# salute-developers/GigaAM

Measured on AMD Instinct MI355X. Metric: RTFx v2_ctc batch32x20s (log-mel + encoder + greedy decode), higher is better.
Workload: dtype f32 (GEMMs: 3-term split on fp16 MFMA, fp32 accumulate)

## Files before the change

### gigaam_amd/_lib.py

```python
from __future__ import annotations

import ctypes as C
import os
from typing import Optional

_HERE = os.path.dirname(os.path.abspath(__file__))
LIB_NAME = "libgigaam_hip.so"
LIB_PATH = os.path.join(_HERE, LIB_NAME)

SUBS_CONV2D, SUBS_CONV1D = 0, 1
ATT_ROTARY, ATT_REL_POS = 0, 1
NORM_BATCH, NORM_LAYER = 0, 1
HEAD_NONE, HEAD_CTC, HEAD_RNNT, HEAD_EMO = 0, 1, 2, 3
DTYPE_F32, DTYPE_F16, DTYPE_BF16, DTYPE_F64, DTYPE_I64 = 0, 1, 2, 3, 4
GEMM_F32, GEMM_F16X3, GEMM_F16 = 0, 1, 2
PF_CLASSES = ["gemm", "conv2", "attn", "norm", "convmod", "stem", "frontend", "decode", "misc", "align_bt", "align_out"]


class GamConfig(C.Structure):
    _fields_ = [(n, C.c_int32) for n in (
        "sample_rate", "n_mels", "hop_length", "win_length", "n_fft", "center",
        "feat_in", "n_layers", "d_model", "subsampling", "subs_kernel_size", "subsampling_factor",
        "ff_expansion_factor", "self_attention_model", "n_heads", "pos_emb_max_len",
        "conv_norm_type", "conv_kernel_size",
# ... 36 lines not shown
    "gam_rnnt_beam_nbest": (C.c_int, [_P, _P, _P, C.c_int, C.c_int64, C.c_int, C.c_int, C.c_int, _P, _P, _P, _P, _P, _P, _P]),
    "gam_op_rnnt_beam_nbest": (C.c_int, [_P, _P, _P, C.c_int, C.c_int64, C.c_int, C.c_int, C.c_int, _P, _P, _P, _P, _P, _P, _P]),
    "gam_rnnt_beam": (C.c_int, [_P, _P, _P, C.c_int, C.c_int64, C.c_int, C.c_int, _P, _P, _P, _P, _P, _P]),
    "gam_op_rnnt_beam": (C.c_int, [_P, _P, _P, C.c_int, C.c_int64, C.c_int, C.c_int, _P, _P, _P, _P, _P, _P]),
    "gam_rnnt_align": (C.c_int, [_P, _P, _P, C.c_int, C.c_int64, _P, _P, C.c_int, _P, _P, _P, _P, _P]),
    "gam_op_rnnt_align": (C.c_int, [_P, _P, _P, C.c_int, C.c_int64, _P, _P, C.c_int, _P, _P, _P, _P, _P, _P]),
    "gam_op_rnnt_lattice_align": (C.c_int, [_P, _P, _P, C.c_int, C.c_int64, C.c_int, _P, _P, C.c_int, _P, _P, _P, _P, _P]),
    "gam_set_rnnt_align_workspace": (C.c_int, [_P, C.c_int64]),
    "gam_ctc_confidence": (C.c_int, [_P, _P, _P, C.c_int, C.c_int64, _P, _P, _P, C.c_int, C.c_int, C.c_int, _P, _P, _P, _P]),
    "gam_op_ctc_confidence": (C.c_int, [_P, _P, _P, C.c_int, C.c_int64, C.c_int, _P, _P, _P, C.c_int, C.c_int, C.c_int, _P, _P, _P, _P]),
    "gam_rnnt_confidence": (C.c_int, [_P, _P, _P, C.c_int, C.c_int64, _P, _P, _P, C.c_int, C.c_int, _P, _P, _P]),
    "gam_op_rnnt_confidence": (C.c_int, [_P, _P, _P, C.c_int, C.c_int64, _P, _P, _P, C.c_int, C.c_int, _P, _P, _P]),
    "gam_emo_probs": (C.c_int, [_P, _P, _P, C.c_int, C.c_int64, _P, _P]),
    "gam_rnnt_predict": (C.c_int, [_P, _P, _P, _P, C.c_int, _P, _P, _P, _P]),
    "gam_rnnt_joint": (C.c_int, [_P, _P, _P, C.c_int, C.c_int, C.c_int, _P, _P]),
    "gam_set_gemm_mode": (C.c_int, [_P, C.c_int]),
    "gam_get_gemm_mode": (C.c_int, [_P]),
    "gam_set_rnnt_cluster": (C.c_int, [_P, C.c_int]),
    "gam_get_rnnt_cluster": (C.c_int, [_P]),
    "gam_debug_buffer_hash": (C.c_int, [_P, C.c_int, C.POINTER(C.c_uint64), C.POINTER(C.c_int64)]),
    "gam_range_flag": (C.c_int, [_P, C.POINTER(C.c_int), _P]),
    "gam_range_flag_fetch": (C.c_int, [_P, _P, _P]),
    "gam_op_gemm": (C.c_int, [_P, _P, _P, _P, _P, C.c_int, C.c_int, C.c_int, C.c_int, _P]),
    "gam_op_attention": (C.c_int, [_P, _P, _P, _P, _P, _P, C.c_int, C.c_int, C.c_int, _P]),
    "gam_op_attention_ex": (C.c_int, [_P, _P, _P, _P, C.c_int64, _P, _P, _P, C.c_int, C.c_int, C.c_int, C.c_int, _P, _P, _P, _P]),
    "gam_tune_sp": (C.c_int, [C.c_int, C.c_int, C.c_int]),
    "gam_plan_sp": (C.c_int, [C.c_int, C.c_int, C.c_int, C.c_int, C.POINTER(C.c_int), C.POINTER(C.c_int), C.POINTER(C.c_int)]),
    "gam_plan_sp_ex": (C.c_int, [C.c_int, C.c_int, C.c_int, C.c_int, C.POINTER(C.c_int), C.POINTER(C.c_int), C.POINTER(C.c_int), C.POINTER(C.c_int)]),
    "gam_tune_sp_stages": (C.c_int, [C.c_int]),
    "gam_profile_enable": (C.c_int, [_P, C.c_int]),
    "gam_profile_pause": (C.c_int, [_P, C.c_int]),
    "gam_profile_read": (C.c_int, [_P, C.c_int, C.POINTER(C.c_double), C.POINTER(C.c_int64), C.POINTER(C.c_double)]),
    "gam_profile_read_bytes": (C.c_int, [_P, C.c_int, C.POINTER(C.c_double)]),
    "gam_last_error": (C.c_char_p, [_P]),
    "gam_comm_unique_id": (C.c_int, [C.c_char_p]),
    "gam_comm_create": (C.c_int, [C.c_char_p, C.c_int, C.c_int, C.c_int, C.POINTER(_P)]),
    "gam_comm_world": (C.c_int, [_P]),
    "gam_gather_ids": (C.c_int, [_P, _P, _P, _P, _P, C.c_int, C.c_int, _P, _P, _P, _P, _P]),
    "gam_comm_last_error": (C.c_char_p, [_P]),
    "gam_comm_destroy": (None, [_P]),
}

_lib: Optional[C.CDLL] = None


class GigaAMHipError(RuntimeError):
# ... 23 lines not shown
```

### gigaam_amd/csrc/gam_api.hip

```cpp
#include <hip/hip_runtime.h>

#include <algorithm>
#include <cmath>
#include <cstdarg>
#include <cstdio>
#include <cstring>
#include <map>
#include <string>
#include <vector>

#include "../../include/gigaam_hip.h"
#include "gam_align.h"
#include "gam_align_long.h"
#include "gam_kws.h"
#include "gam_attn.h"
#include "gam_beam.h"
#include "gam_rnnt_beam.h"
#include "gam_attn16.h"
#include "gam_comm.h"
#include "gam_common.h"
#include "gam_convmod.h"
#include "gam_decode.h"
#include "gam_rnnt_align.h"
#include "gam_confidence.h"
// ... 2294 lines not shown
  ProfScope ps(h, s, GAM_PF_DECODE, (double)rows * V * 8.0);
  hipLaunchKernelGGL(gam_log_softmax_kernel, dim3(gam_cdiv((long)rows, 4)), dim3(256), 0, s, h->jl.p, log_probs, (int)rows, V);
  HIPCHK(h, hipGetLastError());
  return 0;
}

int gam_emo_probs(gam_handle* h, const float* encoded, const int32_t* enc_len, int B, int64_t Tp, float* probs,
                  void* stream) {
  if (!h) return -1;
  if (h->cfg.head_type != GAM_HEAD_EMO || !h->has_head) return fail(h, -1, "model has no emotion head");
  if (B <= 0 || Tp <= 0 || !encoded || !probs) return fail(h, -1, "bad emotion-head arguments");
  HIPCHK(h, hipSetDevice(h->device));
  hipStream_t s = (hipStream_t)stream;
  const int D = h->cfg.d_model, NC = h->cfg.num_classes;
  ProfScope ps(h, s, GAM_PF_DECODE, (double)B * D * Tp * 4.0);
  hipLaunchKernelGGL(gam_emo_head_kernel, dim3(B), dim3(256), (size_t)(D + NC) * sizeof(float), s, encoded, enc_len,
                     h->emo_w, h->emo_b, probs, D, (int)Tp, NC);
  HIPCHK(h, hipGetLastError());
  return 0;
}

int gam_op_gemm(gam_handle* h, const float* A, const float* W, const float* bias, float* C, int M, int N, int K, int act,
                void* stream) {
  if (!h) return -1;
  HIPCHK(h, hipSetDevice(h->device));
  GamGemmArgs g = gemm_args(A, K, W, bias, C, N, M, N, K);
  hipStream_t s = (hipStream_t)stream;
  if (!split_mode(h) || K % 32 != 0 || N % 4 != 0) return gemm(h, s, g, act);
  const size_t wn = (size_t)N * K, an = (size_t)M * K;
  W16 w16;
  if (int r = ensure(h, h->op_sp, wn + 64)) return r;
  hipLaunchKernelGGL(gam_to_sp32_kernel, dim3((int)std::min<size_t>((wn / 4 + 255) / 256, 4096)), dim3(256), 0, s, W,
                     (_Float16*)h->op_sp.p, wn / 4, (const float*)nullptr, K);
  w16.sp = (_Float16*)h->op_sp.p;
  if (int r = ensure(h, h->op_rs, (size_t)M + 64)) return r;
  hipLaunchKernelGGL(gam_rowscale_kernel, dim3(gam_cdiv(M, 4)), dim3(256), 0, s, A, h->op_rs.p, M, K, (long)K);
  g.a_rs = h->op_rs.p;
  if (int r = ensure(h, h->aplanes, an + 64)) return r;
  g.Asp = (const _Float16*)h->aplanes.p;
  g.a_fmt = (h->gemm_mode == GAM_GEMM_F16 && K % 64 == 0) ? 2 : 1;
  if (g.a_fmt == 2) {
    if (int r = ensure(h, h->op_planes, wn / 2 + 64)) return r;
    w16.h16 = (_Float16*)h->op_planes.p;
    hipLaunchKernelGGL(gam_to_h16_kernel, dim3((int)std::min<size_t>((wn / 4 + 255) / 256, 4096)), dim3(256), 0, s, W, w16.h16,
                       wn / 4, (const float*)nullptr, K);
    hipLaunchKernelGGL(gam_to_h16_kernel, dim3((int)std::min<size_t>((an / 4 + 255) / 256, 8192)), dim3(256), 0, s, A,
                       (_Float16*)h->aplanes.p, an / 4, (const float*)h->op_rs.p, K);
  } else {
    hipLaunchKernelGGL(gam_to_sp32_kernel, dim3((int)std::min<size_t>((an / 4 + 255) / 256, 8192)), dim3(256), 0, s, A,
// ... 169 lines not shown
```

### gigaam_amd/csrc/gam_gemm_sp.h

```cpp
#pragma once
#include "gam_gemm.h"
#include <type_traits>
#if defined(GAM_SP_INSTRUMENT) && GAM_SP_INSTRUMENT
#include <algorithm>
#include <vector>
#endif

#ifndef GAM_SP_INSTRUMENT
#define GAM_SP_INSTRUMENT 0
#endif
#define GAM_SP_DBG(g) (GAM_SP_INSTRUMENT ? (g).dbg : 0)
#if GAM_SP_INSTRUMENT
#define GAM_SP_TL(i)                                                                  \
  if ((GAM_SP_DBG(g) & 16) && g.tlog != nullptr && threadIdx.x == 0) {                        \
    g.tlog[(size_t)lid * 8 + (i)] = wall_clock64();                                   \
    if ((i) == 1 || (i) == 2) g.tlog[(size_t)lid * 8 + 4 + (i)] = clock64();          \
    if ((i) == 0) g.tlog[(size_t)lid * 8 + 7] = blockIdx.x;                            \
  }
#else
#define GAM_SP_TL(i)
#endif

template <int MT, int NW, int NS = 2>
struct GamGemmSpCfg {
  static constexpr int BM = 64 * MT;
  static constexpr int BN = 64 * NW;
  static constexpr int NWAVES = 2 * NW;
  static constexpr int NT = 64 * NWAVES;
  static constexpr int A_BYTES = BM * 128;
  static constexpr int W_BYTES = BN * 128;
  static constexpr int STAGE = A_BYTES + W_BYTES;
  static constexpr int SMEM = NS * STAGE;
  static constexpr int NAI = BM / 8 / NWAVES;
  static constexpr int NWI = BN / 8 / NWAVES;
};

template <int ACT, int MT, int NW, int NS = 2, bool H16 = false>
__global__ __launch_bounds__(128 * NW, NW == 2 ? 2 : 1) void gam_gemm_sp_kernel(GamGemmArgs g) {
  extern __shared__ __attribute__((aligned(16))) unsigned char gam_smem_sp[];
  using Cfg = GamGemmSpCfg<MT, NW, NS>;
  constexpr int BM = Cfg::BM, BN = Cfg::BN, NAI = Cfg::NAI, NWI = Cfg::NWI, NWAVES = Cfg::NWAVES;
  typedef __attribute__((address_space(3))) void* lds_ptr_t;
  typedef const __attribute__((address_space(1))) void* glb_ptr_t;

  const int tid = threadIdx.x;
  const int lane = tid & 63;
  const int wave = __builtin_amdgcn_readfirstlane(tid >> 6);
  const int wm = wave / NW, wn = wave % NW;

  const int nbn = (g.N + BN - 1) / BN;
  const int total = gridDim.x;
  const int q8 = total >> 3, r8 = total & 7;
  const int bid = blockIdx.x;
  const int xcd = bid & 7;
  const int lid = (xcd < r8 ? xcd * (q8 + 1) : r8 * (q8 + 1) + (xcd - r8) * q8) + (bid >> 3);
  int tm = lid / nbn, tn = lid % nbn;
  if (g.skip_pad) {
    tm = bid / nbn;
    tn = bid % nbn;
// ... 6 lines not shown
  }
  const int m0 = tm * BM;
  const int n0 = tn * BN;
  if (g.skip_pad && g.lens != nullptr) {
    const int mlast = m0 + BM - 1 < g.M ? m0 + BM - 1 : g.M - 1;
    const int b0 = m0 / g.rpb;
    if (b0 == mlast / g.rpb && (m0 - b0 * g.rpb) / g.fdiv >= g.lens[b0]) return;
  }
  GAM_SP_TL(0);

  auto a_row_off = [&](int m) -> size_t {
    m = m < g.M ? m : g.M - 1;
    if (g.a_mode == 0) return (size_t)m * (size_t)g.lda;
    const int fr = m / g.conv_f2, ff = m - fr * g.conv_f2;
    return ((size_t)fr * 2 * g.conv_fp + 2 * ff) * (size_t)g.conv_c;
  };
  const size_t a_tile0 = a_row_off(m0);
  const unsigned char* Ab = reinterpret_cast<const unsigned char*>(g.n_switch > 0 && n0 >= g.n_switch ? g.Asp2 : g.Asp) + a_tile0 * 4;
  const unsigned char* Wb = reinterpret_cast<const unsigned char*>(g.Wsp) + (size_t)n0 * (size_t)g.K * 4;
  unsigned a_src[NAI], w_src[NWI];
#pragma unroll
  for (int i = 0; i < NAI; ++i) {
    const int row = 8 * (wave + NWAVES * i) + (lane >> 3);
    const int slot = (lane & 7) ^ ((row >> 1) & 7);
    a_src[i] = (unsigned)((a_row_off(m0 + row) - a_tile0) * 4) + slot * 16;
  }
#pragma unroll
  for (int i = 0; i < NWI; ++i) {
    const int row = 8 * (wave + NWAVES * i) + (lane >> 3);
    const int slot = (lane & 7) ^ ((row >> 1) & 7);
    int n = n0 + row;
    n = n < g.N ? n : g.N - 1;
    w_src[i] = (unsigned)(n - n0) * (unsigned)g.K * 4u + slot * 16;
  }

  f32x16 acc[MT][2];
#pragma unroll
  for (int i = 0; i < MT; ++i)
#pragma unroll
    for (int j = 0; j < 2; ++j)
#pragma unroll
      for (int r = 0; r < 16; ++r) acc[i][j][r] = 0.f;

  const int nslice = g.splitk > 1 ? g.splitk : 1;
  const int nk = g.K / 32 / nslice;
  const int kt_first = (nslice > 1 ? (int)blockIdx.y : 0) * nk, kt_end = kt_first + nk;
  int d_kt = kt_first, d_c0 = 0, d_kw = 0, d_kh = 0;
  if (g.a_mode != 0) {
    const int cb = kt_first / 9, t9 = kt_first - cb * 9;
    d_c0 = 32 * cb; d_kh = t9 / 3; d_kw = t9 - d_kh * 3;
  }
  auto dma_ka = [&]() -> size_t {
    if (g.a_mode == 0) return (size_t)d_kt * 128;
    return (((size_t)d_kh * g.conv_fp + d_kw) * (size_t)g.conv_c + d_c0) * 4;
  };
  auto dma_advance = [&]() {
    if (d_kt + 1 >= kt_end) return;
    ++d_kt;
    if (g.a_mode == 0) return;
    if (++d_kw == 3) {
      d_kw = 0;
      if (++d_kh == 3) { d_kh = 0; d_c0 += 32; }
    }
  };
  auto issue = [&](int stage) {
    unsigned char* sb = gam_smem_sp + stage * Cfg::STAGE + wave * 1024;
    const unsigned char* ab = Ab + dma_ka();
    const unsigned char* wb = Wb + (size_t)d_kt * 128;
#pragma unroll
    for (int i = 0; i < NAI; ++i)
      __builtin_amdgcn_global_load_lds((glb_ptr_t)(ab + a_src[i]), (lds_ptr_t)(sb + i * (NWAVES * 1024)), 16, 0, 0);
#pragma unroll
    for (int i = 0; i < NWI; ++i)
      __builtin_amdgcn_global_load_lds((glb_ptr_t)(wb + w_src[i]), (lds_ptr_t)(sb + Cfg::A_BYTES + i * (NWAVES * 1024)), 16, 0, 0);
    dma_advance();
  };

  const int sx = (lane >> 1) & 7;
  const int kg = lane >> 5;
  const int rowb = (lane & 31) * 128;
  const int o_h0 = rowb + (((0 + kg) ^ sx) << 4), o_h1 = rowb + (((2 + kg) ^ sx) << 4);
  const int o_l0 = rowb + (((4 + kg) ^ sx) << 4), o_l1 = rowb + (((6 + kg) ^ sx) << 4);
  const int a_base = wm * (BM / 2) * 128;
  const int w_base = Cfg::A_BYTES + wn * 64 * 128;

  gam_half8 fah[2][MT], fal[2][MT], fbh[2][2], fbl[2][2];
  constexpr int NTERM = H16 ? 2 : 3;
  constexpr int NM = 2 * NTERM * MT;
  constexpr int NR = 2 * MT + 4;
  constexpr int NG = NAI + NWI;
  constexpr int G0 = ((NR + 1) / 2 + NG <= NM) ? (NR + 1) / 2 : 0;
  static_assert((NR + 1) / 2 <= NM && G0 + NG <= NM, "phase too short for its reads + DMA pieces");
#define GAM_SPLD(P) (*reinterpret_cast<const gam_half8*>(P))
#define GAM_SP_RDITEM(S, Q, ST, OH, OL)                                                           \
  {                                                                                               \
    const int q_ = (Q);                                                                           \
    if (q_ < 2) fbh[S][q_ & 1] = GAM_SPLD((ST) + w_base + (q_ & 1) * 4096 + (OH));                 \
    else if (q_ < MT + 2) fah[S][(q_ + MT - 2) % MT] = GAM_SPLD((ST) + a_base + ((q_ + MT - 2) % MT) * 4096 + (OH)); \
    else if (q_ < MT + 4) fbl[S][(q_ - MT) & 1] = GAM_SPLD((ST) + w_base + ((q_ - MT) & 1) * 4096 + (OL)); \
    else fal[S][(q_ + MT - 4) % MT] = GAM_SPLD((ST) + a_base + ((q_ + MT - 4) % MT) * 4096 + (OL)); \
  }
#define GAM_SP_MFMA(S, T)                                                                         \
  {                                                                                               \
    const int term_ = (T) / (2 * MT), i_ = ((T) % (2 * MT)) / 2, j_ = (T) & 1;                    \
     \
    acc[i_][j_] = __builtin_amdgcn_mfma_f32_32x32x16_f16(term_ == 1 ? fbl[S][j_] : fbh[S][j_],    \
                                                         (H16 ? term_ == 1 : term_ == 2) ? fal[S][i_] : fah[S][i_], acc[i_][j_], 0, 0, 0); \
  }
  auto phase = [&](auto setc, auto dmac, const unsigned char* rst, int roh, int rol, int istage) {
    constexpr int S = decltype(setc)::value, R = 1 - S;
    constexpr bool DMA = decltype(dmac)::value;
    const unsigned char* ab = Ab;
    const unsigned char* wb = Wb;
    unsigned char* sb = gam_smem_sp;
    if constexpr (DMA) {
      ab = Ab + dma_ka();
      wb = Wb + (size_t)d_kt * 128;
      sb = gam_smem_sp + istage * Cfg::STAGE + wave * 1024;
      dma_advance();
    }
#pragma unroll
    for (int t = 0; t < NM; ++t) {
      GAM_SP_MFMA(S, t);
      if (2 * t < NR) GAM_SP_RDITEM(R, 2 * t, rst, roh, rol);
      if (2 * t + 1 < NR) GAM_SP_RDITEM(R, 2 * t + 1, rst, roh, rol);
      if (DMA && t >= G0 && t - G0 < NG) {
        const int gi = t - G0;
        if (gi < NAI)
          __builtin_amdgcn_global_load_lds((glb_ptr_t)(ab + a_src[gi % NAI]), (lds_ptr_t)(sb + gi * (NWAVES * 1024)), 16, 0, 0);
        else
          __builtin_amdgcn_global_load_lds((glb_ptr_t)(wb + w_src[(gi - NAI + NWI) % NWI]),
                                           (lds_ptr_t)(sb + Cfg::A_BYTES + (gi - NAI) * (NWAVES * 1024)), 16, 0, 0);
      }
      __builtin_amdgcn_sched_barrier(0);
    }
  };
  using C0_ = std::integral_constant<int, 0>;
  using C1_ = std::integral_constant<int, 1>;
  using T_ = std::integral_constant<bool, true>;
  using F_ = std::integral_constant<bool, false>;

  long long t_bar = 0, t_mm0 = 0, t_mm1 = 0, t_start = 0, w_start = 0;
  if (GAM_SP_DBG(g) & 4) { t_start = clock64(); w_start = wall_clock64(); }
  if (GAM_SP_INSTRUMENT && g.prio && wave >= NWAVES / 2) __builtin_amdgcn_s_setprio(1);
  constexpr int VMW = (NS - 2) * NG;
  static_assert(VMW < 64, "vmcnt field");
#pragma unroll
  for (int st_ = 0; st_ < NS; ++st_) issue(st_);
  if constexpr (NS == 2) {
    __builtin_amdgcn_s_waitcnt(0x0070);
    __syncthreads();
  } else {
    asm volatile("s_waitcnt vmcnt(%0) lgkmcnt(0)\n\ts_barrier" ::"n"(VMW) : "memory");
  }
  GAM_SP_TL(1);
#pragma unroll
  for (int q = 0; q < NR; ++q) GAM_SP_RDITEM(0, q, gam_smem_sp, o_h0, o_l0);
  const int nk_run = (GAM_SP_DBG(g) & 2) ? 1 : nk;
  int s_cur = 0;
  for (int kt = 0; kt < nk_run; ++kt) {
    const int s_nxt = s_cur + 1 == NS ? 0 : s_cur + 1;
    const unsigned char* st = gam_smem_sp + s_cur * Cfg::STAGE;
    const unsigned char* sn = gam_smem_sp + s_nxt * Cfg::STAGE;
    long long c0 = 0, c1 = 0, c2 = 0, c3 = 0;
    if (GAM_SP_DBG(g) & 4) c0 = clock64();
    __builtin_amdgcn_s_waitcnt(0xc07f);
    phase(C0_{}, F_{}, st, o_h1, o_l1, 0);
    if (GAM_SP_DBG(g) & 4) c1 = clock64();
    if constexpr (NS == 2) {
      __builtin_amdgcn_s_waitcnt(0x0070);
      if (!(GAM_SP_DBG(g) & 8)) __syncthreads();
    } else {
      asm volatile("s_waitcnt vmcnt(%0) lgkmcnt(0)\n\ts_barrier" ::"n"(VMW) : "memory");
    }
    if (GAM_SP_DBG(g) & 4) c2 = clock64();
    phase(C1_{}, T_{}, sn, o_h0, o_l0, s_cur);
    if (GAM_SP_DBG(g) & 4) { c3 = clock64(); t_mm0 += c1 - c0; t_bar += c2 - c1; t_mm1 += c3 - c2; }
    s_cur = s_nxt;
  }
  if ((GAM_SP_DBG(g) & 4) && lane == 0 && (lid == 0 || lid == (int)gridDim.x - 1)) {
    float* d = g.C + (size_t)(g.M - 1) * g.ldc + (lid == 0 ? 0 : 64) + wave * 8;
    d[0] = (float)(clock64() - t_start); d[1] = (float)(wall_clock64() - w_start);
    d[2] = (float)t_mm0; d[3] = (float)t_bar; d[4] = (float)t_mm1;
    return;
  }
#undef GAM_SPLD
#undef GAM_SP_RDITEM
#undef GAM_SP_MFMA
  __builtin_amdgcn_s_waitcnt(0x0070);
  GAM_SP_TL(2);

  const int mw = m0 + wm * (BM / 2), nw = n0 + wn * 64;
  if ((GAM_SP_DBG(g) & 1) && acc[0][0][0] != 123.456f) return;

  __builtin_amdgcn_sched_barrier(0);
  asm volatile("s_nop 15\n\ts_nop 15" ::: "memory");
#pragma unroll
  for (int i = 0; i < MT; ++i)
#pragma unroll
    for (int j = 0; j < 2; ++j)
#pragma unroll
      for (int pq = 0; pq < 2; ++pq)
#pragma unroll
        for (int r = 0; r < 4; ++r) {
          float x = acc[i][j][8 * pq + r], y = acc[i][j][8 * pq + 4 + r];
          asm volatile("v_permlane32_swap_b32 %0, %1" : "+v"(x), "+v"(y));
          acc[i][j][8 * pq + r] = x;
          acc[i][j][8 * pq + 4 + r] = y;
        }
  const int lrow = lane & 31, lq8 = (lane >> 5) * 8;
  const float accscale = g.wscale_inv;
  f32x4 bv[2][2][2];
#pragma unroll
  for (int j = 0; j < 2; ++j)
#pragma unroll
    for (int pq = 0; pq < 2; ++pq)
#pragma unroll
      for (int hf = 0; hf < 2; ++hf) {
        const int col = nw + 32 * j + 16 * pq + lq8 + 4 * hf;
        bv[j][pq][hf] = (g.bias != nullptr && col < g.N) ? *reinterpret_cast<const f32x4*>(g.bias + col) : (f32x4){0.f, 0.f, 0.f, 0.f};
      }
#pragma unroll
  for (int i = 0; i < MT; ++i) {
    const int row = mw + 32 * i + lrow;
    if (row >= g.M) continue;
    bool masked = false, skip = false;
    long orow = row;
    if (g.lens != nullptr || g.remap) {
      const int bb = row / g.rpb, tt = row - bb * g.rpb;
      if (g.lens != nullptr) masked = (tt / g.fdiv) >= g.lens[bb];
      if (g.remap) {
        skip = tt >= g.rows_valid;
        orow = (long)bb * g.out_rpb + tt + g.out_shift;
      }
    }
    if (skip && g.partial == nullptr) continue;
    const float rsc = accscale * (g.a_rs != nullptr ? g.a_rs[row] : 1.0f);
    if (g.partial != nullptr) {
      float* P = g.partial + ((size_t)blockIdx.y * (size_t)g.M + (size_t)row) * (size_t)g.N;
#pragma unroll
      for (int j = 0; j < 2; ++j)
#pragma unroll
        for (int pq = 0; pq < 2; ++pq)
#pragma unroll
          for (int hf = 0; hf < 2; ++hf) {
            const int ecol = nw + 32 * j + 16 * pq + lq8 + 4 * hf, r0 = 8 * pq + 4 * hf;
            if (ecol < g.N)
              *reinterpret_cast<f32x4*>(P + ecol) = (f32x4){acc[i][j][r0], acc[i][j][r0 + 1], acc[i][j][r0 + 2], acc[i][j][r0 + 3]} * rsc;
          }
      continue;
    }
    f32x4 rv[2][2][2];
    if (g.R != nullptr) {
#pragma unroll
      for (int j = 0; j < 2; ++j)
#pragma unroll
        for (int pq = 0; pq < 2; ++pq)
#pragma unroll
          for (int hf = 0; hf < 2; ++hf) {
            const int col = nw + 32 * j + 16 * pq + lq8 + 4 * hf;
            rv[j][pq][hf] = col < g.N ? *reinterpret_cast<const f32x4*>(g.R + orow * g.ldr + col) : (f32x4){0.f, 0.f, 0.f, 0.f};
          }
    }
#pragma unroll
    for (int j = 0; j < 2; ++j)
#pragma unroll
      for (int pq = 0; pq < 2; ++pq) {
        const int ecol = nw + 32 * j + 16 * pq + lq8;
        if (ecol >= g.N) continue;
        const bool both = ecol + 4 < g.N;
        f32x4 v[2];
#pragma unroll
        for (int hf = 0; hf < 2; ++hf) {
          const int r0 = 8 * pq + 4 * hf;
          f32x4 t = (f32x4){acc[i][j][r0], acc[i][j][r0 + 1], acc[i][j][r0 + 2], acc[i][j][r0 + 3]};
          t = t * rsc + bv[j][pq][hf];
          if (ACT == GAM_ACT_SILU) { t.x = gam_silu(t.x); t.y = gam_silu(t.y); t.z = gam_silu(t.z); t.w = gam_silu(t.w); }
          if (ACT == GAM_ACT_RELU) { t.x = fmaxf(t.x, 0.f); t.y = fmaxf(t.y, 0.f); t.z = fmaxf(t.z, 0.f); t.w = fmaxf(t.w, 0.f); }
          if (masked) t = (f32x4){0.f, 0.f, 0.f, 0.f};
          t = t * g.alpha;
          if (g.R != nullptr) t += rv[j][pq][hf];
          if (!both && hf == 1) t = (f32x4){0.f, 0.f, 0.f, 0.f};
          v[hf] = t;
        }
        if (g.c_guard) { gam_range_note(g.range_flag, v[0].x, v[0].y, v[0].z, v[0].w); gam_range_note(g.range_flag, v[1].x, v[1].y, v[1].z, v[1].w); }
        if ((GAM_SP_DBG(g) & 32) && v[0].x != 123.456f) continue;
        if (g.c_split == 2) {
          _Float16* cp = reinterpret_cast<_Float16*>(g.C) + orow * g.ldc + ecol;
          const gam_half4 h0 = __builtin_convertvector(v[0], gam_half4), h1 = __builtin_convertvector(v[1], gam_half4);
          if (both) *reinterpret_cast<gam_half8*>(cp) = (gam_half8){h0[0], h0[1], h0[2], h0[3], h1[0], h1[1], h1[2], h1[3]};
          else *reinterpret_cast<gam_half4*>(cp) = h0;
        } else if (g.c_split) {
          _Float16* cp = reinterpret_cast<_Float16*>(g.C) + orow * (2 * g.ldc) + (ecol >> 5) * 64 + (ecol & 31);
          gam_half4 hi0, lo0, hi1, lo1;
          gam_split4(v[0], hi0, lo0);
          gam_split4(v[1], hi1, lo1);
          if (both) {
            *reinterpret_cast<gam_half8*>(cp) = (gam_half8){hi0[0], hi0[1], hi0[2], hi0[3], hi1[0], hi1[1], hi1[2], hi1[3]};
            *reinterpret_cast<gam_half8*>(cp + 32) = (gam_half8){lo0[0], lo0[1], lo0[2], lo0[3], lo1[0], lo1[1], lo1[2], lo1[3]};
          } else {
            *reinterpret_cast<gam_half4*>(cp) = hi0;
            *reinterpret_cast<gam_half4*>(cp + 32) = lo0;
          }
        } else {
          *reinterpret_cast<f32x4*>(g.C + orow * g.ldc + ecol) = v[0];
          if (both) *reinterpret_cast<f32x4*>(g.C + orow * g.ldc + ecol + 4) = v[1];
        }
      }
  }
#if GAM_SP_INSTRUMENT
  if (GAM_SP_DBG(g) & 16) { __builtin_amdgcn_s_waitcnt(0x0070); __syncthreads(); }
  GAM_SP_TL(3);
#endif
}

static inline bool gam_gemm_sp_epilogue_ok(const GamGemmArgs& a) {
  auto al16 = [](const void* p) { return (reinterpret_cast<uintptr_t>(p) & 15) == 0; };
  return a.N % 4 == 0 && a.ldc % 4 == 0 && al16(a.C) && (a.bias == nullptr || al16(a.bias)) &&
         (a.R == nullptr || (a.ldr % 4 == 0 && al16(a.R)));
}

template <int ACT, int MT, int NW, int NS = 2, bool H16 = false>
static inline void gam_launch_gemm_sp_t(const GamGemmArgs& a, int grid, hipStream_t stream) {
  static std::atomic<unsigned long long> attr_devs{0};
  constexpr int smem = GamGemmSpCfg<MT, NW, NS>::SMEM;
  static_assert(smem <= 160 * 1024, "LDS stages do not fit a CU");
  auto kern = gam_gemm_sp_kernel<ACT, MT, NW, NS, H16>;
  if (gam_set_max_lds(reinterpret_cast<const void*>(kern), smem, attr_devs) != hipSuccess) return;
  hipLaunchKernelGGL(kern, dim3(grid, a.splitk > 1 ? a.splitk : 1), dim3(128 * NW), smem, stream, a);
}

struct GamSpPlan { int mt, nw, s, ns; };
// ... 207 lines not shown
```

### gigaam_amd/engine.py

```python
from __future__ import annotations

import ctypes as C
from typing import Any, Dict, Mapping, Optional, Tuple

import numpy as np
import torch
from torch import Tensor

from . import _lib
from ._lib import GamConfig, GigaAMHipError


def _get(cfg: Any, key: str, default: Any = None) -> Any:
    if cfg is None:
        return default
    if isinstance(cfg, Mapping):
        return cfg.get(key, default)
    return getattr(cfg, key, default)


def build_config(pre: Any = None, enc: Any = None, head: Any = None) -> GamConfig:
    c = GamConfig()
    sr = _get(pre, "sample_rate", 16000)
    c.sample_rate = sr
# ... 1056 lines not shown
            h_in, c_in = self._dev(state[0], torch.float32), self._dev(state[1], torch.float32)
            if tuple(h_in.shape) != (nl, b, ph) or tuple(c_in.shape) != (nl, b, ph):
                raise GigaAMHipError(f"predictor state must be two [{nl},{b},{ph}] tensors, got {tuple(h_in.shape)} / {tuple(c_in.shape)}")
        g = torch.empty((b, ph), dtype=torch.float32, device=self.device)
        h_out = torch.empty((nl, b, ph), dtype=torch.float32, device=self.device)
        c_out = torch.empty_like(h_out)
        with torch.cuda.device(self.device):
            rc = self.lib.gam_rnnt_predict(self._h, _ptr(labels), _ptr(h_in), _ptr(c_in), b, _ptr(g), _ptr(h_out), _ptr(c_out), self._stream())
        self._check(rc, "gam_rnnt_predict")
        return g, (h_out, c_out)

    def rnnt_joint(self, enc: Tensor, dec: Tensor) -> Tensor:
        enc, dec = self._dev(enc, torch.float32), self._dev(dec, torch.float32)
        b, t, d = enc.shape
        b2, u, ph = dec.shape
        if b != b2 or d != self.cfg.d_model or ph != self.cfg.pred_hidden:
            raise GigaAMHipError(f"joint expects [B,T,{self.cfg.d_model}] and [B,U,{self.cfg.pred_hidden}], got {tuple(enc.shape)} / {tuple(dec.shape)}")
        out = torch.empty((b, t, u, self.cfg.num_classes), dtype=torch.float32, device=self.device)
        with torch.cuda.device(self.device):
            rc = self.lib.gam_rnnt_joint(self._h, _ptr(enc), _ptr(dec), b, t, u, _ptr(out), self._stream())
        self._check(rc, "gam_rnnt_joint")
        return out

    def op_gemm(self, a: Tensor, w: Tensor, bias: Optional[Tensor] = None, act: int = 0) -> Tensor:
        a = self._dev(a, torch.float32)
        w = self._dev(w, torch.float32)
        bias = None if bias is None else self._dev(bias, torch.float32)
        m, k = a.shape
        n = w.shape[0]
        out = torch.empty((m, n), dtype=torch.float32, device=self.device)
        with torch.cuda.device(self.device):
            rc = self.lib.gam_op_gemm(self._h, _ptr(a), _ptr(w), _ptr(bias), _ptr(out), m, n, k, act, self._stream())
        self._check(rc, "gam_op_gemm")
        return out

    def op_attention(self, q: Tensor, k: Tensor, v: Tensor, lens: Optional[Tensor] = None) -> Tensor:
        q, k, v = (self._dev(t, torch.float32) for t in (q, k, v))
        b, t, d = q.shape
        lens_d = None if lens is None else self._dev(lens, torch.int32)
        out = torch.empty_like(q)
        with torch.cuda.device(self.device):
            rc = self.lib.gam_op_attention(self._h, _ptr(q), _ptr(k), _ptr(v), _ptr(out), _ptr(lens_d), b, t, d // 48, self._stream())
        self._check(rc, "gam_op_attention")
        return out

    def op_attention_ex(self, q: Tensor, k: Tensor, v: Tensor, B: int, Ta: int, Tv: int, H: int, lens: Optional[Tensor] = None,
                        cu: Optional[Tensor] = None, pbuf: Optional[Tensor] = None, pos_u: Optional[Tensor] = None,
                        pos_v: Optional[Tensor] = None) -> Tensor:
        ldq = q.stride(0)
        if not (q.is_cuda and k.is_cuda and v.is_cuda) or k.stride(0) != ldq or v.stride(0) != ldq or any(t.stride(1) != 1 for t in (q, k, v)):
            raise GigaAMHipError("op_attention_ex: q, k, v must be CUDA row views with one row stride")
        lens_d, cu_d = (None if t is None else self._dev(t, torch.int32) for t in (lens, cu))
        pbuf, pos_u, pos_v = (None if t is None else self._dev(t, torch.float32) for t in (pbuf, pos_u, pos_v))
        out = torch.full((q.shape[0], H * 48), float("nan"), dtype=torch.float32, device=self.device)
        with torch.cuda.device(self.device):
            rc = self.lib.gam_op_attention_ex(self._h, _ptr(q), _ptr(k), _ptr(v), ldq, _ptr(out), _ptr(lens_d), _ptr(cu_d), B, Ta, Tv, H,
# ... 20 lines not shown
```

### include/gigaam_hip.h

```cpp
#ifndef GIGAAM_HIP_H
#define GIGAAM_HIP_H

#include <stdint.h>

#ifdef __cplusplus
extern "C" {
#endif

#define GAM_ABI_VERSION 1

typedef struct gam_handle gam_handle;

enum { GAM_SUBS_CONV2D = 0, GAM_SUBS_CONV1D = 1 };
enum { GAM_ATT_ROTARY = 0, GAM_ATT_REL_POS = 1 };
enum { GAM_NORM_BATCH = 0, GAM_NORM_LAYER = 1 };
enum { GAM_HEAD_NONE = 0, GAM_HEAD_CTC = 1, GAM_HEAD_RNNT = 2, GAM_HEAD_EMO = 3 };
enum { GAM_DTYPE_F32 = 0, GAM_DTYPE_F16 = 1, GAM_DTYPE_BF16 = 2, GAM_DTYPE_F64 = 3, GAM_DTYPE_I64 = 4 };

typedef struct gam_config {
  int32_t sample_rate, n_mels, hop_length, win_length, n_fft, center;
  int32_t feat_in, n_layers, d_model, subsampling, subs_kernel_size, subsampling_factor;
  int32_t ff_expansion_factor, self_attention_model, n_heads, pos_emb_max_len;
  int32_t conv_norm_type, conv_kernel_size;
  int32_t head_type, num_classes, pred_hidden, pred_rnn_layers, joint_hidden;
// ... 97 lines not shown
int gam_op_rnnt_confidence(gam_handle* h, const float* encp, const int32_t* enc_len, int B, int64_t Tp, const int32_t* ids,
                           const int32_t* frames, const int32_t* counts, int cap, int measure, float* conf, int32_t* status, void* stream);

int gam_set_rnnt_cluster(gam_handle* h, int workgroups_per_utterance);
int gam_get_rnnt_cluster(gam_handle* h);

int gam_debug_buffer_hash(gam_handle* h, int which, uint64_t* hash_out, int64_t* floats_out);

int gam_rnnt_predict(gam_handle* h, const int32_t* labels, const float* h_in, const float* c_in, int B, float* g_out,
                     float* h_out, float* c_out, void* stream);
int gam_rnnt_joint(gam_handle* h, const float* enc, const float* dec, int B, int T, int U, float* log_probs, void* stream);

int gam_emo_probs(gam_handle* h, const float* encoded, const int32_t* enc_len, int B, int64_t Tp, float* probs,
                  void* stream);

enum { GAM_GEMM_F32 = 0, GAM_GEMM_F16X3 = 1, GAM_GEMM_F16 = 2 };
int gam_set_gemm_mode(gam_handle* h, int mode);
int gam_range_flag(gam_handle* h, int* flag_host, void* stream);
int gam_range_flag_fetch(gam_handle* h, int32_t* flag_dev, void* stream);
int gam_get_gemm_mode(const gam_handle* h);

int gam_op_gemm(gam_handle* h, const float* A, const float* W, const float* bias, float* C,
                int M, int N, int K, int act, void* stream);

int gam_op_attention(gam_handle* h, const float* q, const float* k, const float* v, float* ctx,
                     const int32_t* lens, int B, int T, int H, void* stream);
int gam_op_attention_ex(gam_handle* h, const float* q, const float* k, const float* v, int64_t ldq, float* ctx,
                        const int32_t* lens, const int32_t* cu, int B, int Ta, int Tv, int H, const float* pbuf,
                        const float* pos_u, const float* pos_v, void* stream);

int gam_tune_sp(int mt, int nw, int splitk);
int gam_plan_sp(int M, int N, int K, int n_cu, int* mt, int* nw, int* splitk);
int gam_plan_sp_ex(int M, int N, int K, int n_cu, int* mt, int* nw, int* splitk, int* stages);
int gam_tune_sp_stages(int stages);

enum { GAM_PF_GEMM = 0, GAM_PF_CONV2 = 1, GAM_PF_ATTN = 2, GAM_PF_NORM = 3, GAM_PF_CONVMOD = 4,
       GAM_PF_STEM = 5, GAM_PF_FRONTEND = 6, GAM_PF_DECODE = 7, GAM_PF_MISC = 8,
       GAM_PF_ALIGN_BT = 9, GAM_PF_ALIGN_OUT = 10,
       GAM_PF_NCLASS = 11 };
int gam_profile_enable(gam_handle* h, int on);
int gam_profile_read(gam_handle* h, int cls, double* ms, int64_t* launches, double* work);
int gam_profile_pause(gam_handle* h, int on);
int gam_profile_read_bytes(gam_handle* h, int cls, double* bytes);

typedef struct gam_comm gam_comm;
#define GAM_COMM_ID_BYTES 128
// ... 16 lines not shown
```

Measured before the change: 19310.

## Switch split GEMM to 16x16x32 MFMA tiles with quadrant-scheduled LDS reads

Replaces the 32x32x16 fp16 MFMA tiling in the split-precision GEMM kernel with 16x16x32 MFMAs. The main loop becomes two half passes that interleave LDS fragment reads and async global-to-LDS DMA pieces with the quadrant MFMAs, and the LDS swizzle key changes. This removes the permlane32 swap and s_nop padding from the epilogue. The epilogue now precomputes per-row masking and remap state and prefetches the residual row ahead of use. A gam_op_gemm_ex entry point exposing residual and alpha is added for testing; it risks more MFMA instructions and different register pressure.

```diff
diff --git a/gigaam_amd/_lib.py b/gigaam_amd/_lib.py
--- a/gigaam_amd/_lib.py
+++ b/gigaam_amd/_lib.py
@@ -82,6 +82,7 @@
     "gam_range_flag": (C.c_int, [_P, C.POINTER(C.c_int), _P]),
     "gam_range_flag_fetch": (C.c_int, [_P, _P, _P]),
     "gam_op_gemm": (C.c_int, [_P, _P, _P, _P, _P, C.c_int, C.c_int, C.c_int, C.c_int, _P]),
+    "gam_op_gemm_ex": (C.c_int, [_P, _P, _P, _P, _P, C.c_float, _P, C.c_int, C.c_int, C.c_int, C.c_int, _P]),
     "gam_op_attention": (C.c_int, [_P, _P, _P, _P, _P, _P, C.c_int, C.c_int, C.c_int, _P]),
     "gam_op_attention_ex": (C.c_int, [_P, _P, _P, _P, C.c_int64, _P, _P, _P, C.c_int, C.c_int, C.c_int, C.c_int, _P, _P, _P, _P]),
     "gam_tune_sp": (C.c_int, [C.c_int, C.c_int, C.c_int]),
diff --git a/gigaam_amd/csrc/gam_api.hip b/gigaam_amd/csrc/gam_api.hip
--- a/gigaam_amd/csrc/gam_api.hip
+++ b/gigaam_amd/csrc/gam_api.hip
@@ -2340,9 +2340,15 @@
 
 int gam_op_gemm(gam_handle* h, const float* A, const float* W, const float* bias, float* C, int M, int N, int K, int act,
                 void* stream) {
+  return gam_op_gemm_ex(h, A, W, bias, nullptr, 1.0f, C, M, N, K, act, stream);
+}
+
+int gam_op_gemm_ex(gam_handle* h, const float* A, const float* W, const float* bias, const float* R, float alpha, float* C, int M,
+                   int N, int K, int act, void* stream) {
   if (!h) return -1;
   HIPCHK(h, hipSetDevice(h->device));
   GamGemmArgs g = gemm_args(A, K, W, bias, C, N, M, N, K);
+  g.R = R; g.ldr = N; g.alpha = alpha;
   hipStream_t s = (hipStream_t)stream;
   if (!split_mode(h) || K % 32 != 0 || N % 4 != 0) return gemm(h, s, g, act);
   const size_t wn = (size_t)N * K, an = (size_t)M * K;
diff --git a/gigaam_amd/csrc/gam_gemm_sp.h b/gigaam_amd/csrc/gam_gemm_sp.h
--- a/gigaam_amd/csrc/gam_gemm_sp.h
+++ b/gigaam_amd/csrc/gam_gemm_sp.h
@@ -35,6 +35,8 @@
   static constexpr int NWI = BN / 8 / NWAVES;
 };
 
+__device__ __forceinline__ int gam_sp_key(int row) { return ((row >> 1) & 7) ^ ((row >> 3) & 2); }
+
 template <int ACT, int MT, int NW, int NS = 2, bool H16 = false>
 __global__ __launch_bounds__(128 * NW, NW == 2 ? 2 : 1) void gam_gemm_sp_kernel(GamGemmArgs g) {
   extern __shared__ __attribute__((aligned(16))) unsigned char gam_smem_sp[];
@@ -87,25 +89,25 @@
 #pragma unroll
   for (int i = 0; i < NAI; ++i) {
     const int row = 8 * (wave + NWAVES * i) + (lane >> 3);
-    const int slot = (lane & 7) ^ ((row >> 1) & 7);
+    const int slot = (lane & 7) ^ gam_sp_key(row);
     a_src[i] = (unsigned)((a_row_off(m0 + row) - a_tile0) * 4) + slot * 16;
   }
 #pragma unroll
   for (int i = 0; i < NWI; ++i) {
     const int row = 8 * (wave + NWAVES * i) + (lane >> 3);
-    const int slot = (lane & 7) ^ ((row >> 1) & 7);
+    const int slot = (lane & 7) ^ gam_sp_key(row);
     int n = n0 + row;
     n = n < g.N ? n : g.N - 1;
     w_src[i] = (unsigned)(n - n0) * (unsigned)g.K * 4u + slot * 16;
   }
 
-  f32x16 acc[MT][2];
-#pragma unroll
-  for (int i = 0; i < MT; ++i)
-#pragma unroll
-    for (int j = 0; j < 2; ++j)
-#pragma unroll
-      for (int r = 0; r < 16; ++r) acc[i][j][r] = 0.f;
+  f32x4 acc[2 * MT][4];
+#pragma unroll
+  for (int i = 0; i < 2 * MT; ++i)
+#pragma unroll
+    for (int j = 0; j < 4; ++j)
+#pragma unroll
+      for (int r = 0; r < 4; ++r) acc[i][j][r] = 0.f;
 
   const int nslice = g.splitk > 1 ? g.splitk : 1;
   const int nk = g.K / 32 / nslice;
@@ -141,56 +143,75 @@
     dma_advance();
   };
 
-  const int sx = (lane >> 1) & 7;
-  const int kg = lane >> 5;
-  const int rowb = (lane & 31) * 128;
-  const int o_h0 = rowb + (((0 + kg) ^ sx) << 4), o_h1 = rowb + (((2 + kg) ^ sx) << 4);
-  const int o_l0 = rowb + (((4 + kg) ^ sx) << 4), o_l1 = rowb + (((6 + kg) ^ sx) << 4);
+  const int fi = lane & 15, fg = lane >> 4;
+  const int wr = 8 * (fi >> 2) + (fi & 3);
+  int o_a[2][2], o_w[2][2];
+#pragma unroll
+  for (int pl = 0; pl < 2; ++pl)
+#pragma unroll
+    for (int x = 0; x < 2; ++x) {
+      o_a[pl][x] = fi * 128 + (((4 * pl + fg) ^ gam_sp_key(fi + 16 * x)) << 4);
+      o_w[pl][x] = (wr + 4 * x) * 128 + (((4 * pl + fg) ^ gam_sp_key(wr + 4 * x)) << 4);
+    }
   const int a_base = wm * (BM / 2) * 128;
   const int w_base = Cfg::A_BYTES + wn * 64 * 128;
 
-  gam_half8 fah[2][MT], fal[2][MT], fbh[2][2], fbl[2][2];
+  gam_half8 fah[2 * MT], fal[2 * MT], fwh[4], fwl[4];
   constexpr int NTERM = H16 ? 2 : 3;
-  constexpr int NM = 2 * NTERM * MT;
-  constexpr int NR = 2 * MT + 4;
+  constexpr int QM = 2 * NTERM * MT;
   constexpr int NG = NAI + NWI;
-  constexpr int G0 = ((NR + 1) / 2 + NG <= NM) ? (NR + 1) / 2 : 0;
-  static_assert((NR + 1) / 2 <= NM && G0 + NG <= NM, "phase too short for its reads + DMA pieces");
+  constexpr int G3 = QM - 2 * MT;
+  static_assert(4 + 2 * MT <= QM && G3 + QM - 4 >= NG, "quadrant too short for its reads + DMA pieces");
 #define GAM_SPLD(P) (*reinterpret_cast<const gam_half8*>(P))
-#define GAM_SP_RDITEM(S, Q, ST, OH, OL)                                                           \
+#define GAM_SP_RDW(NH, Q, ST)                                                                     \
   {                                                                                               \
     const int q_ = (Q);                                                                           \
-    if (q_ < 2) fbh[S][q_ & 1] = GAM_SPLD((ST) + w_base + (q_ & 1) * 4096 + (OH));                 \
-    else if (q_ < MT + 2) fah[S][(q_ + MT - 2) % MT] = GAM_SPLD((ST) + a_base + ((q_ + MT - 2) % MT) * 4096 + (OH)); \
-    else if (q_ < MT + 4) fbl[S][(q_ - MT) & 1] = GAM_SPLD((ST) + w_base + ((q_ - MT) & 1) * 4096 + (OL)); \
-    else fal[S][(q_ + MT - 4) % MT] = GAM_SPLD((ST) + a_base + ((q_ + MT - 4) % MT) * 4096 + (OL)); \
-  }
-#define GAM_SP_MFMA(S, T)                                                                         \
+    if (q_ < 2) fwh[2 * (NH) + (q_ & 1)] = GAM_SPLD((ST) + w_base + (NH) * 4096 + o_w[0][q_ & 1]);  \
+    else fwl[2 * (NH) + (q_ & 1)] = GAM_SPLD((ST) + w_base + (NH) * 4096 + o_w[1][q_ & 1]);         \
+  }
+#define GAM_SP_RDA(MH, Q, ST)                                                                     \
   {                                                                                               \
-    const int term_ = (T) / (2 * MT), i_ = ((T) % (2 * MT)) / 2, j_ = (T) & 1;                    \
+    const int q_ = (Q), i_ = (MH) * MT + q_ % MT;                                                 \
+    if (q_ < MT) fah[i_] = GAM_SPLD((ST) + a_base + i_ * 2048 + o_a[0][i_ & 1]);                  \
+    else fal[i_] = GAM_SPLD((ST) + a_base + i_ * 2048 + o_a[1][i_ & 1]);                          \
+  }
+#define GAM_SP_MFMA(MH, NH, T)                                                                    \
+  {                                                                                               \
+    const int term_ = (T) / (2 * MT), i_ = (MH) * MT + ((T) % (2 * MT)) / 2, j_ = 2 * (NH) + ((T) & 1); \
      \
-    acc[i_][j_] = __builtin_amdgcn_mfma_f32_32x32x16_f16(term_ == 1 ? fbl[S][j_] : fbh[S][j_],    \
-                                                         (H16 ? term_ == 1 : term_ == 2) ? fal[S][i_] : fah[S][i_], acc[i_][j_], 0, 0, 0); \
-  }
-  auto phase = [&](auto setc, auto dmac, const unsigned char* rst, int roh, int rol, int istage) {
-    constexpr int S = decltype(setc)::value, R = 1 - S;
-    constexpr bool DMA = decltype(dmac)::value;
-    const unsigned char* ab = Ab;
-    const unsigned char* wb = Wb;
-    unsigned char* sb = gam_smem_sp;
-    if constexpr (DMA) {
-      ab = Ab + dma_ka();
-      wb = Wb + (size_t)d_kt * 128;
-      sb = gam_smem_sp + istage * Cfg::STAGE + wave * 1024;
-      dma_advance();
-    }
-#pragma unroll
-    for (int t = 0; t < NM; ++t) {
-      GAM_SP_MFMA(S, t);
-      if (2 * t < NR) GAM_SP_RDITEM(R, 2 * t, rst, roh, rol);
-      if (2 * t + 1 < NR) GAM_SP_RDITEM(R, 2 * t + 1, rst, roh, rol);
-      if (DMA && t >= G0 && t - G0 < NG) {
-        const int gi = t - G0;
+    acc[i_][j_] = __builtin_amdgcn_mfma_f32_16x16x32_f16(term_ == 1 ? fwl[j_] : fwh[j_],          \
+                                                         (H16 ? term_ == 1 : term_ == 2) ? fal[i_] : fah[i_], acc[i_][j_], 0, 0, 0); \
+  }
+  auto half0 = [&](const unsigned char* st) {
+#pragma unroll
+    for (int t = 0; t < QM; ++t) {
+      GAM_SP_MFMA(0, 0, t);
+      if (t < 4) GAM_SP_RDW(1, t, st)
+      else if (t < 4 + 2 * MT) GAM_SP_RDA(1, t - 4, st)
+      __builtin_amdgcn_sched_barrier(0);
+    }
+#pragma unroll
+    for (int t = 0; t < QM; ++t) {
+      GAM_SP_MFMA(0, 1, t);
+      __builtin_amdgcn_sched_barrier(0);
+    }
+  };
+  auto half1 = [&](const unsigned char* sn, int istage) {
+    const unsigned char* ab = Ab + dma_ka();
+    const unsigned char* wb = Wb + (size_t)d_kt * 128;
+    unsigned char* sb = gam_smem_sp + istage * Cfg::STAGE + wave * 1024;
+    dma_advance();
+#pragma unroll
+    for (int u = 0; u < 2 * QM; ++u) {
+      if (u < QM) {
+        GAM_SP_MFMA(1, 0, u);
+        if (u < 2 * MT) GAM_SP_RDA(0, u, sn)
+      } else {
+        GAM_SP_MFMA(1, 1, u - QM);
+        if (u - QM < 4) GAM_SP_RDW(0, u - QM, sn)
+      }
+      const int gi = u < QM ? u - 2 * MT : (u - QM < 4 ? -1 : G3 + u - QM - 4);
+      if (gi >= 0 && gi < NG) {
         if (gi < NAI)
           __builtin_amdgcn_global_load_lds((glb_ptr_t)(ab + a_src[gi % NAI]), (lds_ptr_t)(sb + gi * (NWAVES * 1024)), 16, 0, 0);
         else
@@ -200,10 +221,6 @@
       __builtin_amdgcn_sched_barrier(0);
     }
   };
-  using C0_ = std::integral_constant<int, 0>;
-  using C1_ = std::integral_constant<int, 1>;
-  using T_ = std::integral_constant<bool, true>;
-  using F_ = std::integral_constant<bool, false>;
 
   long long t_bar = 0, t_mm0 = 0, t_mm1 = 0, t_start = 0, w_start = 0;
   if (GAM_SP_DBG(g) & 4) { t_start = clock64(); w_start = wall_clock64(); }
@@ -220,7 +237,9 @@
   }
   GAM_SP_TL(1);
 #pragma unroll
-  for (int q = 0; q < NR; ++q) GAM_SP_RDITEM(0, q, gam_smem_sp, o_h0, o_l0);
+  for (int q = 0; q < 2 * MT; ++q) GAM_SP_RDA(0, q, gam_smem_sp);
+#pragma unroll
+  for (int q = 0; q < 4; ++q) GAM_SP_RDW(0, q, gam_smem_sp);
   const int nk_run = (GAM_SP_DBG(g) & 2) ? 1 : nk;
   int s_cur = 0;
   for (int kt = 0; kt < nk_run; ++kt) {
@@ -229,8 +248,7 @@
     const unsigned char* sn = gam_smem_sp + s_nxt * Cfg::STAGE;
     long long c0 = 0, c1 = 0, c2 = 0, c3 = 0;
     if (GAM_SP_DBG(g) & 4) c0 = clock64();
-    __builtin_amdgcn_s_waitcnt(0xc07f);
-    phase(C0_{}, F_{}, st, o_h1, o_l1, 0);
+    half0(st);
     if (GAM_SP_DBG(g) & 4) c1 = clock64();
     if constexpr (NS == 2) {
       __builtin_amdgcn_s_waitcnt(0x0070);
@@ -239,7 +257,7 @@
       asm volatile("s_waitcnt vmcnt(%0) lgkmcnt(0)\n\ts_barrier" ::"n"(VMW) : "memory");
     }
     if (GAM_SP_DBG(g) & 4) c2 = clock64();
-    phase(C1_{}, T_{}, sn, o_h0, o_l0, s_cur);
+    half1(sn, s_cur);
     if (GAM_SP_DBG(g) & 4) { c3 = clock64(); t_mm0 += c1 - c0; t_bar += c2 - c1; t_mm1 += c3 - c2; }
     s_cur = s_nxt;
   }
@@ -250,7 +268,8 @@
     return;
   }
 #undef GAM_SPLD
-#undef GAM_SP_RDITEM
+#undef GAM_SP_RDW
+#undef GAM_SP_RDA
 #undef GAM_SP_MFMA
   __builtin_amdgcn_s_waitcnt(0x0070);
   GAM_SP_TL(2);
@@ -258,93 +277,89 @@
   const int mw = m0 + wm * (BM / 2), nw = n0 + wn * 64;
   if ((GAM_SP_DBG(g) & 1) && acc[0][0][0] != 123.456f) return;
 
-  __builtin_amdgcn_sched_barrier(0);
-  asm volatile("s_nop 15\n\ts_nop 15" ::: "memory");
-#pragma unroll
-  for (int i = 0; i < MT; ++i)
-#pragma unroll
-    for (int j = 0; j < 2; ++j)
-#pragma unroll
-      for (int pq = 0; pq < 2; ++pq)
-#pragma unroll
-        for (int r = 0; r < 4; ++r) {
-          float x = acc[i][j][8 * pq + r], y = acc[i][j][8 * pq + 4 + r];
-          asm volatile("v_permlane32_swap_b32 %0, %1" : "+v"(x), "+v"(y));
-          acc[i][j][8 * pq + r] = x;
-          acc[i][j][8 * pq + 4 + r] = y;
+  const int lrow = lane & 15, lq8 = (lane >> 4) * 8;
+  const float accscale = g.wscale_inv;
+  f32x4 bv[2][2];
+#pragma unroll
+  for (int pp = 0; pp < 2; ++pp)
+#pragma unroll
+    for (int hf = 0; hf < 2; ++hf) {
+      const int col = nw + 32 * pp + lq8 + 4 * hf;
+      bv[pp][hf] = (g.bias != nullptr && col < g.N) ? *reinterpret_cast<const f32x4*>(g.bias + col) : (f32x4){0.f, 0.f, 0.f, 0.f};
+    }
+  const bool part = g.partial != nullptr;
+  const bool need_bt = !part && (g.lens != nullptr || g.remap);
+  bool r_ok[2 * MT], r_masked[2 * MT];
+  long r_orow[2 * MT];
+  float r_rsc[2 * MT];
+  int bb = 0, tt = 0;
+  if (need_bt) { bb = (mw + lrow) / g.rpb; tt = (mw + lrow) - bb * g.rpb; }
+#pragma unroll
+  for (int i = 0; i < 2 * MT; ++i) {
+    const int row = mw + 16 * i + lrow;
+    bool ok = row < g.M, masked = false;
+    long orow = row;
+    if (need_bt) {
+      if (i > 0) {
+        tt += 16;
+        if (g.rpb < 16) { bb = row / g.rpb; tt = row - bb * g.rpb; }
+        else if (tt >= g.rpb) { tt -= g.rpb; ++bb; }
+      }
+      if (ok) {
+        if (g.lens != nullptr) masked = tt >= g.lens[bb] * g.fdiv;
+        if (g.remap) {
+          if (tt >= g.rows_valid) ok = false;
+          orow = (long)bb * g.out_rpb + tt + g.out_shift;
         }
-  const int lrow = lane & 31, lq8 = (lane >> 5) * 8;
-  const float accscale = g.wscale_inv;
-  f32x4 bv[2][2][2];
-#pragma unroll
-  for (int j = 0; j < 2; ++j)
-#pragma unroll
-    for (int pq = 0; pq < 2; ++pq)
-#pragma unroll
-      for (int hf = 0; hf < 2; ++hf) {
-        const int col = nw + 32 * j + 16 * pq + lq8 + 4 * hf;
-        bv[j][pq][hf] = (g.bias != nullptr && col < g.N) ? *reinterpret_cast<const f32x4*>(g.bias + col) : (f32x4){0.f, 0.f, 0.f, 0.f};
       }
-#pragma unroll
-  for (int i = 0; i < MT; ++i) {
-    const int row = mw + 32 * i + lrow;
-    if (row >= g.M) continue;
-    bool masked = false, skip = false;
-    long orow = row;
-    if (g.lens != nullptr || g.remap) {
-      const int bb = row / g.rpb, tt = row - bb * g.rpb;
-      if (g.lens != nullptr) masked = (tt / g.fdiv) >= g.lens[bb];
-      if (g.remap) {
-        skip = tt >= g.rows_valid;
-        orow = (long)bb * g.out_rpb + tt + g.out_shift;
-      }
-    }
-    if (skip && g.partial == nullptr) continue;
-    const float rsc = accscale * (g.a_rs != nullptr ? g.a_rs[row] : 1.0f);
-    if (g.partial != nullptr) {
-      float* P = g.partial + ((size_t)blockIdx.y * (size_t)g.M + (size_t)row) * (size_t)g.N;
-#pragma unroll
-      for (int j = 0; j < 2; ++j)
-#pragma unroll
-        for (int pq = 0; pq < 2; ++pq)
-#pragma unroll
-          for (int hf = 0; hf < 2; ++hf) {
-            const int ecol = nw + 32 * j + 16 * pq + lq8 + 4 * hf, r0 = 8 * pq + 4 * hf;
-            if (ecol < g.N)
-              *reinterpret_cast<f32x4*>(P + ecol) = (f32x4){acc[i][j][r0], acc[i][j][r0 + 1], acc[i][j][r0 + 2], acc[i][j][r0 + 3]} * rsc;
-          }
-      continue;
-    }
-    f32x4 rv[2][2][2];
-    if (g.R != nullptr) {
-#pragma unroll
-      for (int j = 0; j < 2; ++j)
-#pragma unroll
-        for (int pq = 0; pq < 2; ++pq)
-#pragma unroll
-          for (int hf = 0; hf < 2; ++hf) {
-            const int col = nw + 32 * j + 16 * pq + lq8 + 4 * hf;
-            rv[j][pq][hf] = col < g.N ? *reinterpret_cast<const f32x4*>(g.R + orow * g.ldr + col) : (f32x4){0.f, 0.f, 0.f, 0.f};
-          }
-    }
-#pragma unroll
-    for (int j = 0; j < 2; ++j)
-#pragma unroll
-      for (int pq = 0; pq < 2; ++pq) {
-        const int ecol = nw + 32 * j + 16 * pq + lq8;
+    }
+    r_rsc[i] = accscale * ((ok && g.a_rs != nullptr) ? g.a_rs[row] : 1.0f);
+    r_ok[i] = ok; r_masked[i] = masked; r_orow[i] = orow;
+  }
+  if (part) {
+#pragma unroll
+    for (int i = 0; i < 2 * MT; ++i) {
+      if (!r_ok[i]) continue;
+      float* P = g.partial + ((size_t)blockIdx.y * (size_t)g.M + (size_t)(mw + 16 * i + lrow)) * (size_t)g.N;
+#pragma unroll
+      for (int pp = 0; pp < 2; ++pp)
+#pragma unroll
+        for (int hf = 0; hf < 2; ++hf) {
+          const int ecol = nw + 32 * pp + lq8 + 4 * hf;
+          if (ecol < g.N) *reinterpret_cast<f32x4*>(P + ecol) = acc[i][2 * pp + hf] * r_rsc[i];
+        }
+    }
+  }
+#define GAM_SP_LDR(I, D)                                                                          \
+  _Pragma("unroll") for (int pp = 0; pp < 2; ++pp) _Pragma("unroll") for (int hf = 0; hf < 2; ++hf) { \
+    const int col = nw + 32 * pp + lq8 + 4 * hf;                                                  \
+    D[pp][hf] = (r_ok[I] && col < g.N) ? *reinterpret_cast<const f32x4*>(g.R + r_orow[I] * g.ldr + col) : (f32x4){0.f, 0.f, 0.f, 0.f}; \
+  }
+  f32x4 rv[2][2], rn[2][2];
+  const bool resid = g.R != nullptr && !part;
+  if (resid) GAM_SP_LDR(0, rv);
+#pragma unroll
+  for (int i = 0; i < 2 * MT; ++i) {
+    if (resid && i + 1 < 2 * MT) GAM_SP_LDR(i + 1, rn);
+    const bool masked = r_masked[i];
+    const long orow = r_orow[i];
+    const float rsc = r_rsc[i];
+    if (r_ok[i] && !part) {
+#pragma unroll
+      for (int pp = 0; pp < 2; ++pp) {
+        const int ecol = nw + 32 * pp + lq8;
         if (ecol >= g.N) continue;
         const bool both = ecol + 4 < g.N;
         f32x4 v[2];
 #pragma unroll
         for (int hf = 0; hf < 2; ++hf) {
-          const int r0 = 8 * pq + 4 * hf;
-          f32x4 t = (f32x4){acc[i][j][r0], acc[i][j][r0 + 1], acc[i][j][r0 + 2], acc[i][j][r0 + 3]};
-          t = t * rsc + bv[j][pq][hf];
+          f32x4 t = acc[i][2 * pp + hf];
+          t = t * rsc + bv[pp][hf];
           if (ACT == GAM_ACT_SILU) { t.x = gam_silu(t.x); t.y = gam_silu(t.y); t.z = gam_silu(t.z); t.w = gam_silu(t.w); }
           if (ACT == GAM_ACT_RELU) { t.x = fmaxf(t.x, 0.f); t.y = fmaxf(t.y, 0.f); t.z = fmaxf(t.z, 0.f); t.w = fmaxf(t.w, 0.f); }
           if (masked) t = (f32x4){0.f, 0.f, 0.f, 0.f};
           t = t * g.alpha;
-          if (g.R != nullptr) t += rv[j][pq][hf];
+          if (resid) t += rv[pp][hf];
           if (!both && hf == 1) t = (f32x4){0.f, 0.f, 0.f, 0.f};
           v[hf] = t;
         }
@@ -372,7 +387,15 @@
           if (both) *reinterpret_cast<f32x4*>(g.C + orow * g.ldc + ecol + 4) = v[1];
         }
       }
-  }
+    }
+    if (resid && i + 1 < 2 * MT) {
+#pragma unroll
+      for (int pp = 0; pp < 2; ++pp)
+#pragma unroll
+        for (int hf = 0; hf < 2; ++hf) rv[pp][hf] = rn[pp][hf];
+    }
+  }
+#undef GAM_SP_LDR
 #if GAM_SP_INSTRUMENT
   if (GAM_SP_DBG(g) & 16) { __builtin_amdgcn_s_waitcnt(0x0070); __syncthreads(); }
   GAM_SP_TL(3);
diff --git a/gigaam_amd/engine.py b/gigaam_amd/engine.py
--- a/gigaam_amd/engine.py
+++ b/gigaam_amd/engine.py
@@ -1102,16 +1102,19 @@
         self._check(rc, "gam_rnnt_joint")
         return out
 
-    def op_gemm(self, a: Tensor, w: Tensor, bias: Optional[Tensor] = None, act: int = 0) -> Tensor:
+    def op_gemm(self, a: Tensor, w: Tensor, bias: Optional[Tensor] = None, act: int = 0, resid: Optional[Tensor] = None,
+                alpha: float = 1.0) -> Tensor:
         a = self._dev(a, torch.float32)
         w = self._dev(w, torch.float32)
         bias = None if bias is None else self._dev(bias, torch.float32)
+        resid = None if resid is None else self._dev(resid, torch.float32)
         m, k = a.shape
         n = w.shape[0]
         out = torch.empty((m, n), dtype=torch.float32, device=self.device)
         with torch.cuda.device(self.device):
-            rc = self.lib.gam_op_gemm(self._h, _ptr(a), _ptr(w), _ptr(bias), _ptr(out), m, n, k, act, self._stream())
-        self._check(rc, "gam_op_gemm")
+            rc = self.lib.gam_op_gemm_ex(self._h, _ptr(a), _ptr(w), _ptr(bias), _ptr(resid), alpha, _ptr(out), m, n, k, act,
+                                         self._stream())
+        self._check(rc, "gam_op_gemm_ex")
         return out
 
     def op_attention(self, q: Tensor, k: Tensor, v: Tensor, lens: Optional[Tensor] = None) -> Tensor:
diff --git a/include/gigaam_hip.h b/include/gigaam_hip.h
--- a/include/gigaam_hip.h
+++ b/include/gigaam_hip.h
@@ -143,6 +143,8 @@
 
 int gam_op_gemm(gam_handle* h, const float* A, const float* W, const float* bias, float* C,
                 int M, int N, int K, int act, void* stream);
+int gam_op_gemm_ex(gam_handle* h, const float* A, const float* W, const float* bias, const float* R, float alpha,
+                   float* C, int M, int N, int K, int act, void* stream);
 
 int gam_op_attention(gam_handle* h, const float* q, const float* k, const float* v, float* ctx,
                      const int32_t* lens, int B, int T, int H, void* stream);
```

After: 20260, median of 6. +4.9%, better.
